# lich0031/AIDE

Hardware: AMD Instinct MI355X
Metric: training images/sec FuseUNet 256x256x2 bs=4/GPU (higher is better)
Workload: dtype f32; 1 GPU; c2 fuseunet fwd+loss+bwd+Adam(amsgrad), 256x256 2-modal, bs=4/GPU, fp32; global_batch=4, parallelism=dp1

## Files before the change

aide_amd/csrc/conv3x3_wino4.hip:

```cpp
#include "common.h"
#include <stdlib.h>
#include <type_traits>

namespace {

template <int V> using ic = std::integral_constant<int, V>;

__device__ __forceinline__ void buf_store_f32x4(f32x4 v, __amdgpu_buffer_rsrc_t r, unsigned voff, unsigned soff) {
    __builtin_amdgcn_raw_buffer_store_b128(__builtin_bit_cast(u32x4, v), r, voff, soff, 0);
}
__device__ __forceinline__ void buf_store_f32x2(f32x2 v, __amdgpu_buffer_rsrc_t r, unsigned voff, unsigned soff) {
    __builtin_amdgcn_raw_buffer_store_b64(__builtin_bit_cast(u32x2, v), r, voff, soff, 0);
}

struct W4Args {
    const float* x;
    const float* u;
    const float* bias;
    float* y;
    long x_bs, y_bs, split_stride;
    int N, Cin, H, W, Cout;
    int blocks_w, blocks_h, n_co_tiles, splitk, stages_total, accumulate;
    int gp, gc;
    int pair;
    float* stats;
    const float* scale;
    int relu;
    const float* in_tab;
    int in_ng;
};

constexpr int F4_BNIN_MAXC = 1024;
constexpr int F4_NAGPR = 16;
constexpr int F4_RRS = 41;
constexpr int F4_RCS = 775;
constexpr int F4_RAW = 4 * F4_RCS;
constexpr int F4_V = 36 * 32 * 4;
constexpr int F4_SET = F4_RAW + F4_V;
constexpr int F4_LDS = 2 * F4_SET > 4 * 128 * 64 ? 2 * F4_SET : 4 * 128 * 64;

__host__ __device__ constexpr int f4_pos(int q, int b) {
    return 6 * (q / 3) + ((q % 3) == 0 ? 1 + b : (q % 3) == 1 ? 3 + b : 5 * b);
}
__host__ __device__ constexpr int f4_slot(int c) { return c == 0 ? 4 : c == 5 ? 5 : c - 1; }

__device__ __forceinline__ void bt6(float d0, float d1, float d2, float d3, float d4, float d5, float* o, int st) {
    const float a = __builtin_fmaf(-4.f, d2, d4), b = __builtin_fmaf(4.f, d1, -d3);
    const float c = d4 - d2, e = d3 - d1;
    o[0] = __builtin_fmaf(-5.f, d2, __builtin_fmaf(4.f, d0, d4));
    o[st] = a - b;
    o[2 * st] = a + b;
    o[3 * st] = __builtin_fmaf(2.f, e, c);
    o[4 * st] = __builtin_fmaf(-2.f, e, c);
    o[5 * st] = __builtin_fmaf(-5.f, d3, __builtin_fmaf(4.f, d1, d5));
}

template <int CTRL, int ROW_MASK>
__device__ __forceinline__ float dpp_add(float v) {
    return v + __builtin_bit_cast(float, __builtin_amdgcn_update_dpp(0, __builtin_bit_cast(int, v), CTRL, ROW_MASK, 0xf, true));
}
__device__ __forceinline__ float half_total_dpp(float v) {
    v = dpp_add<0x111, 0xf>(v);
    v = dpp_add<0x112, 0xf>(v);
    v = dpp_add<0x114, 0xf>(v);
    v = dpp_add<0x118, 0xf>(v);
    v = dpp_add<0x142, 0xa>(v);
    return v;
}

template <int MODE, bool AFF = false, bool BNIN = false>
__global__ __launch_bounds__(256, 1) void conv3x3_wino4_kernel(const W4Args a) {
    extern __shared__ __attribute__((aligned(16))) float lds[];
    const int wid = __builtin_amdgcn_readfirstlane((int)threadIdx.x >> 6);
    const int ph = wid & 1, cb = wid >> 1;
    const int hs = wid >> 1;

    int b = xcd_remap(blockIdx.x, gridDim.x);
    const int p_in = b % a.gp;            b /= a.gp;
    const int co_in = b % a.gc;           b /= a.gc;
    const int ncg = a.n_co_tiles / a.gc;
    const int cog = b % ncg;              b /= ncg;
    const int split = b % a.splitk;       b /= a.splitk;
    const int co_tile = cog * a.gc + co_in;
    int pt = b * a.gp + p_in;
    const int tw = pt % a.blocks_w;       pt /= a.blocks_w;
    const int th = pt % a.blocks_h;
    const int n = pt / a.blocks_h;
    constexpr int PAIR = MODE == 1;
    constexpr bool canv = MODE == 2;
    constexpr int NR = canv ? 22 : 18, NI = canv ? 5 : 8, RRS = canv ? 29 : F4_RRS;
    constexpr int TPH = canv ? 20 : 16, TPW = canv ? 20 : 32;
    static_assert(NR * RRS <= F4_RCS, "raw channel plane");
    const int h0 = th * TPH, w0 = tw * TPW, co0 = co_tile * 64;
    const int HW = a.H * a.W;
    constexpr int pair = PAIR;

    const int sps = a.stages_total / a.splitk;
    const int s_begin = split * sps;
    const int s_end = min(s_begin + sps, a.stages_total);

    const __amdgpu_buffer_rsrc_t xrs =
        make_rsrc(a.x + (long)(pair ? 2 * n : n) * a.x_bs + (long)h0 * a.W + w0 - (a.W + 1));
    const long ubase = ((long)9 * ph * 2 * a.Cout + co0 + cb * 32) * 4;
    const __amdgpu_buffer_rsrc_t urs = __builtin_amdgcn_make_buffer_rsrc(
        const_cast<float*>(a.u + ubase), 0, (int)(((long)a.Cin * 36 * a.Cout - ubase) * 4), 0x00020000);
    const unsigned upos = (unsigned)a.Cout * 32u;
    const unsigned upos18 = 18u * upos;
    auto run = [&](auto HS) {
    int lane;
    asm volatile("; lane id, transform half %1\n\tv_mbcnt_lo_u32_b32 %0, -1, 0\n\tv_mbcnt_hi_u32_b32 %0, -1, %0"
                 : "=v"(lane) : "n"(decltype(HS)::value));
    const int tid = wid * 64 + lane;
    const int half = lane >> 5, j = lane & 31;
    constexpr int NUI = 4 * NR * NI, NUE = 4 * NR * 2;
    unsigned offB[3], ldsB[3], offC, ldsC;
    int tabB[3], tabC;
#pragma unroll
    for (int e = 0; e < 3; ++e) {
        int q = tid + e * 256;
        while (q >= NUI) q -= 256;
        const int c = q / (NR * NI), rem = q - c * (NR * NI), r = rem / NI, s4 = rem - r * NI;
        const int ih = h0 - 1 + r, iw = w0 + 4 * s4;
        const int imgB = pair && s4 >= 4;
        const bool ok = ih >= 0 && ih < a.H && (pair || iw < a.W);
        offB[e] = ok ? (unsigned)((long)imgB * a.x_bs + c * HW + r * a.W + 1 + 4 * (pair ? (s4 & 3) : s4)) * 4u : BUF_OOB;
        ldsB[e] = (unsigned)(c * F4_RCS + r * RRS + 4 + 4 * s4 + 2 * imgB);
        tabB[e] = F4_LDS + (ok ? 0 : 2 * a.Cin) + 2 * c;
    }
    {
        int q = tid;
        if (q >= NUE) q -= NUE;
        const int c = q / (NR * 2), rem = q - c * (NR * 2), r = rem >> 1, side = rem & 1;
        const int ih = h0 - 1 + r, iw = side ? w0 + TPW : w0 - 1;
        const bool ok = !pair && ih >= 0 && ih < a.H && iw >= 0 && iw < a.W;
        tabC = F4_LDS + (ok ? 0 : 2 * a.Cin) + 2 * c;
        offC = ok ? (unsigned)(c * HW + r * a.W + (side ? TPW + 1 : 0)) * 4u : BUF_OOB;
        ldsC = (unsigned)(c * F4_RCS + r * RRS + (pair ? (side ? 21 : 20) : (side ? 4 + TPW : 3)));
    }
#pragma unroll
    for (int e = 0; e < 3; ++e) asm volatile("" : "+v"(ldsB[e]), "+v"(offB[e]));
    asm volatile("" : "+v"(ldsC), "+v"(offC));
    const unsigned uoff = (unsigned)(half * a.Cout + j) * 16u;

    f32x4 rb[3];
    float rc;
    f32x4 ua[2][9];
    auto fetch_u = [&](int q, int stage, f32x4* dst) {
        const unsigned us = (unsigned)min(stage, s_end - 1) * upos18 + (unsigned)q * upos;
        dst[q] = buf_load_f32x4(urs, uoff, us);
    };
    auto fetch = [&](int l, int stage) {
        const unsigned xs = (unsigned)(min(stage, s_end - 1) * 4) * (unsigned)HW * 4u;
        if (l < 3) rb[l] = buf_load_f32x4(xrs, offB[l], xs);
        else rc = buf_load_f32(xrs, offC, xs);
    };
    auto put_raw = [&](int w, float* raw) {
        if (w < 12) raw[ldsB[w >> 2] + (w & 3)] = rb[w >> 2][w & 3];
        else raw[ldsC] = rc;
    };
    f32x2 tv[4];
    auto bn_tab = [&](int stage) {
        const int so = min(stage, s_end - 1) * 8;
#pragma unroll
        for (int e = 0; e < 3; ++e) tv[e] = *reinterpret_cast<const f32x2*>(lds + tabB[e] + so);
        tv[3] = *reinterpret_cast<const f32x2*>(lds + tabC + so);
    };
    auto bn_in = [&]() {
#pragma unroll
        for (int e = 0; e < 3; ++e) {
            const f32x2 sc = f32x2{tv[e].x, tv[e].x}, sh = f32x2{tv[e].y, tv[e].y};
            const f32x2 lo = f32x2{rb[e].x, rb[e].y} * sc + sh, hi = f32x2{rb[e].z, rb[e].w} * sc + sh;
            rb[e] = f32x4{fmaxf(lo.x, 0.f), fmaxf(lo.y, 0.f), fmaxf(hi.x, 0.f), fmaxf(hi.y, 0.f)};
        }
        rc = fmaxf(__builtin_fmaf(rc, tv[3].x, tv[3].y), 0.f);
    };
    if constexpr (BNIN) {
        float* tab = lds + F4_LDS;
        const float* src = a.in_tab + (long)(n / a.in_ng) * 2 * a.Cin;
        for (int i = tid; i < 2 * a.Cin; i += 256) { tab[i] = src[i]; tab[2 * a.Cin + i] = 0.f; }
        __syncthreads();
    }

    const int item = tid & 127;
    const int tslot = canv ? min(item >> 2, 24) : (item >> 2);
    const int trow = canv ? tslot / 5 : tslot >> 3, tcol = canv ? tslot - 5 * trow : tslot & 7;
    const int xr_off = (item & 3) * F4_RCS + trow * 4 * RRS + 3 + 4 * tcol + ((pair && tcol >= 4) ? 2 : 0);
    f32x2 tp[6][3];
    f32x2 tq[9];
    auto xf_read = [&](int i, int xo) {
        const float v = lds[xo + (i / 6) * RRS + (i % 6)];
        if ((i % 6) & 1) tp[i / 6][(i % 6) >> 1].y = v; else tp[i / 6][(i % 6) >> 1].x = v;
    };
    auto xf_half = [&](auto HS) {
        constexpr int khs = decltype(HS)::value;
        f32x2 T[3][3];
#pragma unroll
        for (int cp = 0; cp < 3; ++cp) {
            const f32x2 d0 = tp[0][cp], d1 = tp[1][cp], d2 = tp[2][cp], d3 = tp[3][cp], d4 = tp[4][cp], d5 = tp[5][cp];
            if (khs == 0) {
                const f32x2 aa = d4 - 4.f * d2, bb = 4.f * d1 - d3;
                T[0][cp] = (4.f * d0 + d4) - 5.f * d2;
                T[1][cp] = bb * f32x2{-1.f, -1.f} + aa;
                T[2][cp] = aa + bb;
            } else {
                const f32x2 cc = d2 * f32x2{-1.f, -1.f} + d4, ee = d1 * f32x2{-1.f, -1.f} + d3;
                T[0][cp] = cc + 2.f * ee;
                T[1][cp] = cc - 2.f * ee;
                T[2][cp] = (4.f * d1 + d5) - 5.f * d3;
            }
        }
#pragma unroll
        for (int i = 0; i < 3; ++i) {
            const f32x2 t01 = T[i][0], t23 = T[i][1], t45 = T[i][2];
            const f32x2 ac = f32x2{t23.x, t23.x} * f32x2{-4.f, -1.f} + f32x2{t45.x, t45.x};
            const f32x2 be = f32x2{t01.y, t01.y} * f32x2{-4.f, -1.f} + f32x2{t23.y, t23.y};
            const f32x2 o12 = f32x2{be.x, be.x} * f32x2{1.f, -1.f} + f32x2{ac.x, ac.x};
            const f32x2 o34 = f32x2{be.y, be.y} * f32x2{2.f, -2.f} + f32x2{ac.y, ac.y};
            const f32x2 o05 = t23 * f32x2{-5.f, -5.f} + (t01 * f32x2{4.f, 4.f} + t45);
            tq[3 * i] = o12; tq[3 * i + 1] = o34; tq[3 * i + 2] = o05;
        }
    };
    auto xf_math = [&]() { xf_half(HS); };
    const int vitem = ((item >> 1) & 1) * 128 + ((((item >> 2) * 4 + (item & 1) * 2)) ^ (((item >> 1) & 1) * 16));
    auto xf_store = [&](int m, float* vbuf) {
        *reinterpret_cast<f32x2*>(vbuf + (9 * hs + m) * 256 + vitem) = tq[m];
    };

    f32x16 acc[18];
    f32x4 fb[3];

    float* const set0 = lds;
    float* const set1 = lds + F4_SET;
    int xr0 = xr_off, xr1 = F4_SET + xr_off;
    asm volatile("" : "+v"(xr0), "+v"(xr1));
#pragma unroll
    for (int l = 0; l < 4; ++l) fetch(l, s_begin);
#pragma unroll
    for (int q = 0; q < 9; ++q) fetch_u(q, s_begin, ua[0]);
    __builtin_amdgcn_sched_barrier(0);
#pragma unroll
    for (int p = 0; p < 18; ++p) {
#pragma unroll
        for (int r = 0; r < 16; ++r) {
            float z;
            if (p < F4_NAGPR) asm volatile("v_accvgpr_write_b32 %0, 0" : "=a"(z));
            else asm volatile("v_mov_b32 %0, 0" : "=v"(z));
            acc[p][r] = z;
        }
    }
    __builtin_amdgcn_sched_barrier(0);
    if (pair) {
        for (int q = tid; q < 2 * 4 * 18 * 2; q += 256) {
            const int set = q / 144, rem = q - set * 144, c = rem / 36, rr = (rem % 36) >> 1, side = rem & 1;
            lds[set * F4_SET + c * F4_RCS + rr * F4_RRS + (side ? 38 : 3)] = 0.f;
        }
    }
    if constexpr (BNIN) { bn_tab(s_begin); bn_in(); }
#pragma unroll
    for (int w = 0; w < 13; ++w) put_raw(w, set0);
#pragma unroll
    for (int l = 0; l < 4; ++l) fetch(l, s_begin + 1);
    __syncthreads();
#pragma unroll
    for (int i = 0; i < 36; ++i) xf_read(i, xr0);
    xf_math();
#pragma unroll
    for (int m = 0; m < 9; ++m) xf_store(m, set0 + F4_RAW);
    if constexpr (BNIN) { bn_tab(s_begin + 1); bn_in(); }
#pragma unroll
    for (int w = 0; w < 13; ++w) put_raw(w, set1);
    __syncthreads();

    auto stage = [&](int s, float* sc, float* sn, auto CUR) {
        constexpr int kcur = decltype(CUR)::value;
        const float* lb = sc + F4_RAW + (9 * ph) * 256 + half * 128 + ((j * 4) ^ (half * 16));
        auto frag = [&](int q, int slot3) { fb[slot3] = *reinterpret_cast<const f32x4*>(lb + q * 256); };
        frag(0, 0); frag(1, 1);
#pragma unroll
        for (int st = 0; st < 36; ++st) {
            const int g = st >> 2, w = st & 3, pi = 2 * g + (w & 1), k = w >> 1;
            const int fs = g % 3;
            if (w == 0 && g + 2 < 9) frag(g + 2, (g + 2) % 3);
            if (pi < F4_NAGPR) asm volatile("v_mfma_f32_32x32x2_f32 %0, %1, %2, %0" : "+a"(acc[pi]) : "v"(ua[kcur][g][(w & 1) * 2 + k]), "v"(fb[fs][k * 2 + (w & 1)]));
            else asm volatile("v_mfma_f32_32x32x2_f32 %0, %1, %2, %0" : "+v"(acc[pi]) : "v"(ua[kcur][g][(w & 1) * 2 + k]), "v"(fb[fs][k * 2 + (w & 1)]));
            if (st < 4) fetch(st, s + 2);
            else if (st < 22 && ((st - 4) & 1) == 0) fetch_u((st - 4) >> 1, s + 1, ua[1 - kcur]);
            constexpr int XM = 20, XS = 21, PR = 31;
            if (st < 18) { xf_read(2 * st, kcur ? xr0 : xr1); xf_read(2 * st + 1, kcur ? xr0 : xr1); }
            if (st == XM) xf_math();
            if (st >= XS && st < XS + 9) xf_store(st - XS, sn + F4_RAW);
            if constexpr (BNIN) {
                if (st == 24) bn_tab(s + 2);
                if (st == 30) bn_in();
            }
            if (st >= PR && st < PR + 5) {
#pragma unroll
                for (int q = 0; q < 3; ++q)
                    if (3 * (st - PR) + q < 13) put_raw(3 * (st - PR) + q, sc);
            }
            __builtin_amdgcn_sched_barrier(0);
        }
        __syncthreads();
    };
    for (int s = s_begin; s < s_end; s += 2) {
        stage(s, set0, set1, ic<0>{});
        stage(s + 1, set1, set0, ic<1>{});
    }

    float* xbuf = lds;
    const int el = (int)__builtin_amdgcn_mbcnt_hi(~0u, __builtin_amdgcn_mbcnt_lo(~0u, 0u));
    const int eh = el >> 5, ej = el & 31;
    int ez;
    asm volatile("s_mov_b32 %0, 0" : "=s"(ez));
    const int cw = co0 + cb * 32 + ez;
    const bool wlive = cw < a.Cout;
    const bool add_bias = (a.bias != nullptr) && (split == 0);
    const __amdgpu_buffer_rsrc_t yrs = __builtin_amdgcn_make_buffer_rsrc(
        a.y + (long)split * a.split_stride + (long)(pair ? 2 * n : n) * a.y_bs + ez, 0, wlive ? (int)BUF_OOB : 0, 0x00020000);
    const __amdgpu_buffer_rsrc_t brs = __builtin_amdgcn_make_buffer_rsrc(
        const_cast<float*>(a.bias) + ez, 0, (add_bias && wlive) ? a.Cout * 4 : 0, 0x00020000);
    const int oh = h0 + 4 * (canv ? ej / 5 : ej >> 3), ow = pair ? 4 * (ej & 3) : w0 + 4 * (canv ? ej % 5 : ej & 7);
    const bool pok = (!canv || ej < 25) && oh < a.H && ow < a.W;
    const unsigned yoff = pok ? ((pair ? (unsigned)((ej & 7) >> 2) * (unsigned)a.y_bs : 0u) +
                                 (unsigned)(4 * eh * HW + oh * a.W + ow)) * 4u : BUF_OOB;
    const unsigned boff = (unsigned)eh * 16u;
    const int nparts = a.N * a.blocks_h * a.blocks_w;
    const __amdgpu_buffer_rsrc_t srs = __builtin_amdgcn_make_buffer_rsrc(
        a.stats + ez, 0, (a.stats != nullptr && wlive) ? a.Cout * nparts * 8 : 0, 0x00020000);
    const unsigned soff = ej == 31 ? (unsigned)(4 * eh * nparts + (n * a.blocks_h + th) * a.blocks_w + tw) * 8u : BUF_OOB;
    auto epilogue = [&](auto PH) {
        constexpr int kph = decltype(PH)::value;
        auto partial = [&](int r, f32x2* yp) {
            f32x2 T[3][4];
#pragma unroll
            for (int i = 0; i < 3; ++i) {
                auto m = [&](int c) { return f32x2{acc[6 * i + f4_slot(c)][r], acc[6 * i + f4_slot(c)][r + 1]}; };
                const f32x2 m0 = m(0), m1 = m(1), m2 = m(2), m3 = m(3), m4 = m(4), m5 = m(5);
                const f32x2 s12 = m1 + m2, d12 = m2 * f32x2{-1.f, -1.f} + m1, s34 = m3 + m4, d34 = m4 * f32x2{-1.f, -1.f} + m3;
                T[i][0] = m0 + s12 + s34;
                T[i][1] = d34 * f32x2{2.f, 2.f} + d12;
                T[i][2] = s34 * f32x2{4.f, 4.f} + s12;
                T[i][3] = d34 * f32x2{8.f, 8.f} + d12 + m5;
            }
#pragma unroll
            for (int bq = 0; bq < 4; ++bq) {
                if (kph == 0) {
                    const f32x2 sm = T[1][bq] + T[2][bq], df = T[2][bq] * f32x2{-1.f, -1.f} + T[1][bq];
                    yp[bq] = T[0][bq] + sm; yp[4 + bq] = df; yp[8 + bq] = sm; yp[12 + bq] = df;
                } else {
                    const f32x2 sm = T[0][bq] + T[1][bq], df = T[1][bq] * f32x2{-1.f, -1.f} + T[0][bq];
                    yp[bq] = sm; yp[4 + bq] = df * f32x2{2.f, 2.f}; yp[8 + bq] = sm * f32x2{4.f, 4.f};
                    yp[12 + bq] = df * f32x2{8.f, 8.f} + T[2][bq];
                }
            }
        };
        f32x2* const xbuf2 = reinterpret_cast<f32x2*>(xbuf);
#pragma unroll
        for (int rp = 0; rp < 4; ++rp) {
            f32x2 yp[16];
            partial(2 * rp + 8 * (1 - kph), yp);
#pragma unroll
            for (int o = 0; o < 16; ++o) xbuf2[((wid * 64) + rp * 16 + o) * 64 + el] = yp[o];
        }
        float bvs[8], svs[8];
#pragma unroll
        for (int q = 0; q < 8; ++q) {
            const int r = q + 8 * kph;
            bvs[q] = buf_load_f32(brs, boff, (unsigned)(cw + (r & 3) + 8 * (r >> 2)) * 4u);
        }
        if constexpr (AFF) {
            const __amdgpu_buffer_rsrc_t ars = __builtin_amdgcn_make_buffer_rsrc(const_cast<float*>(a.scale), 0, wlive ? a.Cout * 4 : 0, 0x00020000);
#pragma unroll
            for (int q = 0; q < 8; ++q) {
                const int r = q + 8 * kph;
                svs[q] = buf_load_f32(ars, boff, (unsigned)(cw + (r & 3) + 8 * (r >> 2)) * 4u);
            }
        }
        __syncthreads();
#pragma unroll
        for (int rp = 0; rp < 4; ++rp) {
            f32x2 yp[16];
            partial(2 * rp + 8 * kph, yp);
#pragma unroll
            for (int o = 0; o < 16; ++o) yp[o] += xbuf2[(((wid ^ 1) * 64) + rp * 16 + o) * 64 + el];
#pragma unroll
            for (int e = 0; e < 2; ++e) {
                const int r = 2 * rp + e + 8 * kph;
                const unsigned crow = (unsigned)(cw + (r & 3) + 8 * (r >> 2));
                if (a.stats) {
                    float s1 = 0.f, s2 = 0.f;
                    if (pok) {
#pragma unroll
                        for (int o = 0; o < 16; ++o) { s1 += yp[o][e]; s2 = __builtin_fmaf(yp[o][e], yp[o][e], s2); }
                    }
                    s1 = half_total_dpp(s1);
                    s2 = half_total_dpp(s2);
                    buf_store_f32x2(f32x2{s1, s2}, srs, soff, crow * (unsigned)nparts * 8u);
                }
                const float bv = bvs[2 * rp + e];
                const unsigned srow = crow * (unsigned)HW * 4u;
                f32x4 o[4];
#pragma unroll
                for (int i = 0; i < 4; ++i)
                    o[i] = f32x4{yp[4 * i][e] + bv, yp[4 * i + 1][e] + bv, yp[4 * i + 2][e] + bv, yp[4 * i + 3][e] + bv};
                if constexpr (AFF) {
                    const float sv = svs[2 * rp + e];
#pragma unroll
                    for (int i = 0; i < 4; ++i) {
#pragma unroll
                        for (int k = 0; k < 4; ++k) {
                            const float v = __builtin_fmaf(yp[4 * i + k][e], sv, bv);
                            o[i][k] = a.relu ? fmaxf(v, 0.f) : v;
                        }
                    }
                }
                if (a.accumulate) {
                    f32x4 old[4];
#pragma unroll
                    for (int i = 0; i < 4; ++i) old[i] = buf_load_f32x4(yrs, yoff, srow + (unsigned)(i * a.W) * 4u);
#pragma unroll
                    for (int i = 0; i < 4; ++i) o[i] += old[i];
                }
#pragma unroll
                for (int i = 0; i < 4; ++i) buf_store_f32x4(o[i], yrs, yoff, srow + (unsigned)(i * a.W) * 4u);
            }
        }
    };
    if (ph == 0) epilogue(ic<0>{}); else epilogue(ic<1>{});
    };
    if (hs == 0) run(ic<0>{}); else run(ic<1>{});
}

__global__ __launch_bounds__(256) void w4_splitk_reduce_kernel(const float* __restrict__ slabs, long split_stride,
                                                               int splitk, float* __restrict__ y, long y_bs, int C,
                                                               int HW, const float* __restrict__ bias, int accumulate,
                                                               long total4, const float* __restrict__ scale, int relu) {
    for (long i = (long)blockIdx.x * 256 + threadIdx.x; i < total4; i += (long)gridDim.x * 256) {
        const long e = i * 4, chw = (long)C * HW;
        const long n = e / chw, rem = e - n * chw;
        f32x4 v = *reinterpret_cast<const f32x4*>(slabs + e);
        for (int s = 1; s < splitk; ++s) v += *reinterpret_cast<const f32x4*>(slabs + (long)s * split_stride + e);
        if (scale) {
            const float sv = scale[rem / HW], bv = bias[rem / HW];
#pragma unroll
            for (int k = 0; k < 4; ++k) { const float t = __builtin_fmaf(v[k], sv, bv); v[k] = relu ? fmaxf(t, 0.f) : t; }
        } else if (bias) { const float bv = bias[rem / HW]; v += f32x4{bv, bv, bv, bv}; }
        f32x4* p = reinterpret_cast<f32x4*>(y + n * y_bs + rem);
        if (accumulate) v += *p;
        *p = v;
    }
}

__device__ __forceinline__ void wino4_g(const float g[9], float u[36]) {
    float t[18];
#pragma unroll
    for (int c = 0; c < 3; ++c) {
        const float g0 = g[c], g1 = g[3 + c], g2 = g[6 + c];
        const float s = g0 + g2;
        t[c] = 0.25f * g0;
        t[3 + c] = (-1.f / 6.f) * (s + g1);
        t[6 + c] = (-1.f / 6.f) * (s - g1);
        const float q = __builtin_fmaf(4.f, g2, g0);
        t[9 + c] = (1.f / 24.f) * (q + 2.f * g1);
        t[12 + c] = (1.f / 24.f) * (q - 2.f * g1);
        t[15 + c] = g2;
    }
#pragma unroll
    for (int r = 0; r < 6; ++r) {
        const float a0 = t[r * 3], a1 = t[r * 3 + 1], a2 = t[r * 3 + 2];
        const float s = a0 + a2, q = __builtin_fmaf(4.f, a2, a0);
        u[r * 6] = 0.25f * a0;
        u[r * 6 + 1] = (-1.f / 6.f) * (s + a1);
        u[r * 6 + 2] = (-1.f / 6.f) * (s - a1);
        u[r * 6 + 3] = (1.f / 24.f) * (q + 2.f * a1);
        u[r * 6 + 4] = (1.f / 24.f) * (q - 2.f * a1);
        u[r * 6 + 5] = a2;
    }
}

struct W4PackDesc {
    const float* w; float* uf; float* ud;
    int Co, Ci, pad0, pad1;
    long block_start;
};

constexpr int P4_T = 32;
__global__ __launch_bounds__(128) void wino4_pack_multi_kernel(const W4PackDesc* __restrict__ descs, int n, long total_blocks) {
    __shared__ __attribute__((aligned(16))) float ot[36 * 128];
    for (long blk = blockIdx.x; blk < total_blocks; blk += gridDim.x) {
    int lo = 0, hi = n - 1;
    while (lo < hi) {
        const int mid = (lo + hi + 1) >> 1;
        if (descs[mid].block_start <= blk) lo = mid; else hi = mid - 1;
    }
    const W4PackDesc d = descs[lo];
    const int tid = threadIdx.x;
    const int tiles_ci = (d.Ci + P4_T - 1) / P4_T;
    const int tb = (int)(blk - d.block_start);
    const int co0 = (tb / tiles_ci) * P4_T, ci0 = (tb % tiles_ci) * P4_T;
    const int nci = min(P4_T, d.Ci - ci0);
    float g[9], u[36];
    const int lo2 = tid & 3, hi5 = tid >> 2;
    for (int grp = 0; grp < 16; ++grp) {
        const bool fwd = grp < 8;
        const int q = grp & 7;
        float* dst = fwd ? d.uf : d.ud;
        if (dst == nullptr) continue;
        const int co = fwd ? hi5 : 4 * q + lo2, ci = fwd ? 4 * q + lo2 : hi5;
        const bool live = fwd ? (ci0 + 4 * q < d.Ci) : (co0 + 4 * q < d.Co);
        if (!live) continue;
        {
            const bool in = co0 + co < d.Co && ci < nci;
            const float* wp = d.w + ((long)(co0 + co) * d.Ci + ci0 + ci) * 9;
#pragma unroll
            for (int t = 0; t < 9; ++t) g[t] = in ? wp[fwd ? t : 8 - t] : 0.f;
        }
        wino4_g(g, u);
        const int otid = (lo2 >> 1) * 64 + hi5 * 2 + (lo2 & 1);
#pragma unroll
        for (int p = 0; p < 36; ++p) ot[p * 128 + otid] = u[p];
        __syncthreads();
        const int C = fwd ? d.Co : d.Ci, c0 = fwd ? co0 : ci0;
        const long gbase = (long)((fwd ? ci0 : co0) / 4 + q) * 18;
        const int nrow = min(P4_T, C - c0);
#pragma unroll
        for (int k = 0; k < 9; ++k) {
            const int f = tid + k * 128, pq = f >> 6, hh = (f >> 5) & 1, row = f & 31;
            if (row < nrow) {
                const float* o0 = ot + f4_pos(pq, 0) * 128 + hh * 64 + row * 2;
                const float* o1 = ot + f4_pos(pq, 1) * 128 + hh * 64 + row * 2;
                *reinterpret_cast<f32x4*>(dst + (((gbase + pq) * 2 + hh) * C + c0 + row) * 4) =
                    f32x4{o0[0], o0[1], o1[0], o1[1]};
            }
        }
        __syncthreads();
    }
    }
}

}

extern "C" {

int aide_conv3x3_wino4_supported(int Cin, int H, int W, int Cout) {
    return (H % 4 == 0 && W % 4 == 0 && H >= 16 && W >= 16 && Cout % 32 == 0 &&
            Cin % 8 == 0) ? 1 : 0;
}

static int f4_mode(int H, int W, int* bh, int* bw) {
    const int sh = (H + 15) / 16, sw = (W + 31) / 32, ch = (H + 19) / 20, cw = (W + 19) / 20;
    const int mode = W == 16 ? 1 : ((long)ch * cw < (long)sh * sw) ? 2 : 0;
    *bh = mode == 2 ? ch : sh;
    *bw = mode == 2 ? cw : sw;
    return mode;
}

int aide_conv3x3_wino4_splitk(int N, int Cin, int H, int W, int Cout) {
    int bh, bw;
    f4_mode(H, W, &bh, &bw);
    const long nb = (long)bh * bw * (W == 16 ? N / 2 : N) * ((Cout + 63) / 64);
    const int pairs = Cin / 8;
    const long target = 200;
    int s = 1;
    while (nb * s < target && pairs % (s * 2) == 0 && s * 2 <= pairs / 4) s *= 2;
    return s;
}

int aide_conv3x3_wino4_stats_parts(int N, int H, int W) {
    int bh, bw;
    f4_mode(H, W, &bh, &bw);
    return W < 32 ? 0 : N * bh * bw;
}

int aide_conv3x3_wino4_pack_blocks(int Co, int Ci) {
    return ((Co + P4_T - 1) / P4_T) * ((Ci + P4_T - 1) / P4_T);
}

int aide_conv3x3_wino4_pack_multi(const void* descs, int n, int64_t total_blocks, hipStream_t stream) {
    if (!descs || n <= 0 || total_blocks <= 0) return AIDE_ERR_ARG;
    static_assert(sizeof(W4PackDesc) == 48, "descriptor layout");
    const long grid = total_blocks;
    AIDE_LAUNCH_TIMED(AIDE_KT_OTHER, 0.0, wino4_pack_multi_kernel, dim3((unsigned)grid), dim3(128), 0, stream,
                       (const W4PackDesc*)descs, n, (long)total_blocks);
    return aide_launch_status();
}

int aide_conv3x3_wino4(const float* x, int64_t x_bs, const float* u, const float* bias, float* y,
                       int64_t y_bs, int N, int Cin, int H, int W, int Cout, int accumulate, int splitk,
                       float* ws, float* stats_parts, const float* epi_scale, int epi_relu, const float* in_bn_tab,
                       int in_bn_group_images, hipStream_t stream) {
    const float* aff = epi_scale;
    const int aff_relu = aff ? epi_relu : 0;
    if (!x || !u || !y || !aide_conv3x3_wino4_supported(Cin, H, W, Cout) || x_bs % 4 || y_bs % 4 || (W == 16 && N % 2))
        return AIDE_ERR_ARG;
    static AideLdsOptIn lds_opt;
    if (int rc = lds_opt.ensure([] {
            constexpr int plain = F4_LDS * (int)sizeof(float), bnin = (F4_LDS + 4 * F4_BNIN_MAXC) * (int)sizeof(float);
            const struct { const void* fn; int bytes; } ks[] = {
                {(const void*)conv3x3_wino4_kernel<0>, plain}, {(const void*)conv3x3_wino4_kernel<1>, plain},
                {(const void*)conv3x3_wino4_kernel<2>, plain}, {(const void*)conv3x3_wino4_kernel<0, true>, plain},
                {(const void*)conv3x3_wino4_kernel<2, true>, plain}, {(const void*)conv3x3_wino4_kernel<0, false, true>, bnin},
                {(const void*)conv3x3_wino4_kernel<2, false, true>, bnin}};
            for (const auto& k : ks) {
                const hipError_t e = hipFuncSetAttribute(k.fn, hipFuncAttributeMaxDynamicSharedMemorySize, k.bytes);
                if (e != hipSuccess) return e;
            }
            return hipSuccess;
        })) return rc;
    W4Args a;
    if (stats_parts && !(splitk <= 1 && accumulate == 0 && W >= 32)) return AIDE_ERR_ARG;
    a.stats = stats_parts;
    const int mode = f4_mode(H, W, &a.blocks_h, &a.blocks_w);
    if (aff && (accumulate != 0 || !bias || (mode == 1 && splitk <= 1))) return AIDE_ERR_ARG;
    a.scale = splitk > 1 ? nullptr : aff;
    a.relu = aff_relu;
    a.pair = mode == 1 ? 1 : 0;
    if (in_bn_tab && (mode == 1 || aff || Cin > F4_BNIN_MAXC || in_bn_group_images < 1 || N % in_bn_group_images)) return AIDE_ERR_ARG;
    a.in_tab = in_bn_tab; a.in_ng = in_bn_tab ? in_bn_group_images : 1;
    a.x = x; a.u = u; a.x_bs = x_bs; a.N = N; a.Cin = Cin; a.H = H; a.W = W; a.Cout = Cout;
    a.n_co_tiles = (Cout + 63) / 64;
    a.stages_total = Cin / 4;
    if (splitk < 1) splitk = 1;
    if ((Cin / 8) % splitk != 0) return AIDE_ERR_ARG;
    if (splitk > 1 && !ws) return AIDE_ERR_ARG;
    a.splitk = splitk;
    if (splitk > 1) {
        a.y = ws; a.y_bs = (long)Cout * H * W; a.split_stride = (long)N * Cout * H * W;
        a.bias = nullptr; a.accumulate = 0;
    } else {
        a.y = y; a.y_bs = y_bs; a.split_stride = 0; a.bias = bias; a.accumulate = (accumulate == 1);
    }
    if (((a.pair ? a.y_bs : 0) + (long)Cout * H * W) * 4 >= (1L << 31)) return AIDE_ERR_ARG;
    if (a.stats && (long)Cout * N * a.blocks_h * a.blocks_w * 8 >= (1L << 31)) return AIDE_ERR_ARG;
    const long nb = (long)a.blocks_w * a.blocks_h * (a.pair ? N / 2 : N) * a.n_co_tiles * splitk;
    {
        const long P = (long)a.blocks_w * a.blocks_h * (a.pair ? N / 2 : N);
        const int C = a.n_co_tiles;
        const long per_xcd = nb / 8 > 0 ? nb / 8 : 1;
        const double ub = 144.0 * (double)Cin * Cout, xb = 1.44 * 4.0 * (double)N * Cin * H * W;
        long bp = 1; int bc = C;
        double best = 1e300;
        const bool grouped = AIDE_CONV_FLOPS(N, H, W, Cout, Cin) >= 8e9;
        for (long gp = 1; gp <= P && gp <= per_xcd && grouped; gp *= 2) {
            if (P % gp) continue;
            for (int gc = 1; gc <= C; ++gc) {
                if (C % gc || gp * gc > per_xcd) continue;
                const double cost = ub * (double)P / (double)gp + xb * (double)C / (double)gc;
                if (cost < best) { best = cost; bp = gp; bc = gc; }
            }
        }
        a.gp = (int)bp; a.gc = bc;
    }
    if (a.in_tab) {
        const size_t lds_bytes = (F4_LDS + 4 * (size_t)Cin) * sizeof(float);
        if (mode == 2) {
            AIDE_LAUNCH_TIMED(AIDE_KT_WINO4, AIDE_CONV_FLOPS(N, H, W, Cout, Cin), (conv3x3_wino4_kernel<2, false, true>),
                              dim3((unsigned)nb), dim3(256), lds_bytes, stream, a);
        } else {
            AIDE_LAUNCH_TIMED(AIDE_KT_WINO4, AIDE_CONV_FLOPS(N, H, W, Cout, Cin), (conv3x3_wino4_kernel<0, false, true>),
                              dim3((unsigned)nb), dim3(256), lds_bytes, stream, a);
        }
    } else if (a.scale && mode == 2) {
        AIDE_LAUNCH_TIMED(AIDE_KT_WINO4, AIDE_CONV_FLOPS(N, H, W, Cout, Cin), (conv3x3_wino4_kernel<2, true>), dim3((unsigned)nb),
                          dim3(256), F4_LDS * sizeof(float), stream, a);
    } else if (a.scale) {
        AIDE_LAUNCH_TIMED(AIDE_KT_WINO4, AIDE_CONV_FLOPS(N, H, W, Cout, Cin), (conv3x3_wino4_kernel<0, true>), dim3((unsigned)nb),
                          dim3(256), F4_LDS * sizeof(float), stream, a);
    } else if (a.pair) {
        AIDE_LAUNCH_TIMED(AIDE_KT_WINO4, AIDE_CONV_FLOPS(N, H, W, Cout, Cin), conv3x3_wino4_kernel<1>, dim3((unsigned)nb), dim3(256),
                          F4_LDS * sizeof(float), stream, a);
    } else if (mode == 2) {
        AIDE_LAUNCH_TIMED(AIDE_KT_WINO4, AIDE_CONV_FLOPS(N, H, W, Cout, Cin), conv3x3_wino4_kernel<2>, dim3((unsigned)nb), dim3(256),
                          F4_LDS * sizeof(float), stream, a);
    } else {
        AIDE_LAUNCH_TIMED(AIDE_KT_WINO4, AIDE_CONV_FLOPS(N, H, W, Cout, Cin), conv3x3_wino4_kernel<0>, dim3((unsigned)nb), dim3(256),
                          F4_LDS * sizeof(float), stream, a);
    }
    int rc = aide_launch_status();
    if (rc != 0) return rc;
    if (splitk > 1 && accumulate != 2) {
        const long total4 = (long)N * Cout * H * W / 4;
        AIDE_LAUNCH_TIMED(AIDE_KT_REDUCE, 0.0, w4_splitk_reduce_kernel, dim3((unsigned)min((total4 + 255) / 256, 4096L)), dim3(256), 0,
                           stream, ws, (long)N * Cout * H * W, splitk, y, (long)y_bs, Cout, H * W, bias, accumulate,
                           total4, aff, aff_relu);
        rc = aide_launch_status();
    }
    return rc;
}

}
```

Baseline: 655.6 images/sec.

## Move stage barrier inside the Winograd MFMA loop and prefetch next-stage fragments

Restructures the software pipeline of the F(4,3) Winograd conv kernel. The per-stage __syncthreads now sits at slot 31 of the 36-slot MFMA schedule instead of at the end. The first two V fragments of the next stage are loaded after that barrier, so MFMAs can keep issuing across the stage boundary. Raw-input global fetches move later and run three stages ahead, and raw LDS stores and BN steps are rescheduled earlier, with static_asserts checking the slot ordering. This hides the barrier and fragment-load latency at the cost of more register pressure and a deeper global prefetch, whose out-of-range stage index must be handled safely.

```diff
diff --git a/aide_amd/csrc/conv3x3_wino4.hip b/aide_amd/csrc/conv3x3_wino4.hip
--- a/aide_amd/csrc/conv3x3_wino4.hip
+++ b/aide_amd/csrc/conv3x3_wino4.hip
@@ -38,6 +38,49 @@
 constexpr int F4_V = 36 * 32 * 4;
 constexpr int F4_SET = F4_RAW + F4_V;
 constexpr int F4_LDS = 2 * F4_SET > 4 * 128 * 64 ? 2 * F4_SET : 4 * 128 * 64;
+
+constexpr int W4_SLOTS = 36, W4_PAIRS = 9;
+constexpr int W4_FB = 3;
+constexpr int W4_AHEAD = 2;
+constexpr int W4_XR = 0, W4_XR_N = 18;
+constexpr int W4_UF = 4;
+constexpr int W4_XM = 20;
+constexpr int W4_XS = 21;
+constexpr int W4_BT = 19, W4_BI = 23;
+constexpr int W4_PR = 24, W4_PR_N = 5;
+constexpr int W4_RF = 29, W4_RF_N = 4;
+constexpr int W4_BAR = 31;
+constexpr int W4_PF0 = 31, W4_PF1 = 32;
+constexpr int w4_frag_slot(int q) { return 4 * (q - W4_AHEAD); }
+constexpr int w4_last_use(int g) { return 4 * g + 3; }
+constexpr int w4_last_pair_of(int f) {
+    int g = -1;
+    for (int q = 0; q < W4_PAIRS; ++q) if (q % W4_FB == f) g = q;
+    return g;
+}
+constexpr bool w4_fb_rotation_ok() {
+    for (int q = W4_AHEAD; q < W4_PAIRS; ++q) {
+        if (w4_frag_slot(q) < 0 || w4_frag_slot(q) >= 4 * q) return false;
+        if (q >= W4_FB && w4_frag_slot(q) <= w4_last_use(q - W4_FB)) return false;
+    }
+    return true;
+}
+static_assert(W4_BAR > 0 && W4_BAR < W4_SLOTS, "one barrier per stage, inside it");
+static_assert(w4_frag_slot(W4_PAIRS - 1) < W4_BAR, "sc.V is read in front of the barrier: the next interval overwrites it");
+static_assert(W4_PF0 >= W4_BAR && W4_PF1 >= W4_BAR && W4_PF0 < W4_SLOTS && W4_PF1 < W4_SLOTS,
+              "sn.V is read behind the barrier that follows its stores");
+static_assert(W4_XS >= W4_XM && W4_XS + W4_PAIRS - 1 < W4_BAR, "sn.V is written in front of the barrier");
+static_assert(W4_XR >= 0 && W4_XR + W4_XR_N - 1 < W4_BAR, "sn.raw is read in front of the barrier: the next interval overwrites it");
+static_assert(W4_PR >= 0 && W4_PR + W4_PR_N - 1 < W4_BAR, "sc.raw is written in front of the barrier, its readers follow behind it");
+static_assert(3 * W4_PR_N >= 13 && 2 * W4_XR_N == 36, "13 raw words, 36 patch words per thread");
+static_assert(W4_XM > W4_XR + W4_XR_N - 1, "the transform follows the last patch read");
+static_assert(W4_RF > W4_PR + W4_PR_N - 1 && W4_RF + W4_RF_N <= W4_SLOTS, "the raw registers are refilled behind their LDS stores");
+static_assert(W4_BT < W4_BI && W4_BI <= W4_PR && W4_BI != W4_XM, "BNIN: table, then the activation, then the raw stores");
+static_assert(W4_UF + 2 * (W4_PAIRS - 1) < W4_RF, "nine filter fetches per stage, in slots of their own");
+static_assert(W4_AHEAD == 2 && W4_FB == 3 && w4_fb_rotation_ok(), "fragment q: requested at slot 4 (q - 2) into fb[q % 3]");
+static_assert(W4_PF0 > w4_last_use(w4_last_pair_of(0)) && W4_PF1 > w4_last_use(w4_last_pair_of(1)),
+              "the next stage's fragments 0 / 1 go into fb[0] / fb[1] behind the last pair that used them");
+static_assert(W4_PF0 != W4_PF1, "one prefetch per slot");
 
 __host__ __device__ constexpr int f4_pos(int q, int b) {
     return 6 * (q / 3) + ((q % 3) == 0 ? 1 + b : (q % 3) == 1 ? 3 + b : 5 * b);
@@ -227,12 +270,14 @@
     };
 
     f32x16 acc[18];
-    f32x4 fb[3];
+    f32x4 fb[W4_FB];
 
     float* const set0 = lds;
     float* const set1 = lds + F4_SET;
     int xr0 = xr_off, xr1 = F4_SET + xr_off;
     asm volatile("" : "+v"(xr0), "+v"(xr1));
+    const int vfrag = (9 * ph) * 256 + half * 128 + ((j * 4) ^ (half * 16));
+    auto frag = [&](int q, const float* set) { fb[q % W4_FB] = *reinterpret_cast<const f32x4*>(set + F4_RAW + vfrag + q * 256); };
 #pragma unroll
     for (int l = 0; l < 4; ++l) fetch(l, s_begin);
 #pragma unroll
@@ -269,43 +314,48 @@
     if constexpr (BNIN) { bn_tab(s_begin + 1); bn_in(); }
 #pragma unroll
     for (int w = 0; w < 13; ++w) put_raw(w, set1);
+#pragma unroll
+    for (int l = 0; l < 4; ++l) fetch(l, s_begin + 2);
     __syncthreads();
+#pragma unroll
+    for (int q = 0; q < W4_AHEAD; ++q) frag(q, set0);
 
     auto stage = [&](int s, float* sc, float* sn, auto CUR) {
         constexpr int kcur = decltype(CUR)::value;
-        const float* lb = sc + F4_RAW + (9 * ph) * 256 + half * 128 + ((j * 4) ^ (half * 16));
-        auto frag = [&](int q, int slot3) { fb[slot3] = *reinterpret_cast<const f32x4*>(lb + q * 256); };
-        frag(0, 0); frag(1, 1);
-#pragma unroll
-        for (int st = 0; st < 36; ++st) {
+#pragma unroll
+        for (int st = 0; st < W4_SLOTS; ++st) {
             const int g = st >> 2, w = st & 3, pi = 2 * g + (w & 1), k = w >> 1;
-            const int fs = g % 3;
-            if (w == 0 && g + 2 < 9) frag(g + 2, (g + 2) % 3);
+            const int fs = g % W4_FB;
+            if (st == W4_BAR) __syncthreads();
+            if (w == 0 && g + W4_AHEAD < W4_PAIRS) frag(g + W4_AHEAD, sc);
+            if (st == W4_PF0) frag(0, sn);
+            if (st == W4_PF1) frag(1, sn);
             if (pi < F4_NAGPR) asm volatile("v_mfma_f32_32x32x2_f32 %0, %1, %2, %0" : "+a"(acc[pi]) : "v"(ua[kcur][g][(w & 1) * 2 + k]), "v"(fb[fs][k * 2 + (w & 1)]));
             else asm volatile("v_mfma_f32_32x32x2_f32 %0, %1, %2, %0" : "+v"(acc[pi]) : "v"(ua[kcur][g][(w & 1) * 2 + k]), "v"(fb[fs][k * 2 + (w & 1)]));
-            if (st < 4) fetch(st, s + 2);
-            else if (st < 22 && ((st - 4) & 1) == 0) fetch_u((st - 4) >> 1, s + 1, ua[1 - kcur]);
-            constexpr int XM = 20, XS = 21, PR = 31;
-            if (st < 18) { xf_read(2 * st, kcur ? xr0 : xr1); xf_read(2 * st + 1, kcur ? xr0 : xr1); }
-            if (st == XM) xf_math();
-            if (st >= XS && st < XS + 9) xf_store(st - XS, sn + F4_RAW);
+            if (st >= W4_RF && st < W4_RF + W4_RF_N) fetch(st - W4_RF, s + 3);
+            else if (st >= W4_UF && st < W4_UF + 2 * W4_PAIRS && ((st - W4_UF) & 1) == 0) fetch_u((st - W4_UF) >> 1, s + 1, ua[1 - kcur]);
+            if (st >= W4_XR && st < W4_XR + W4_XR_N) {
+                xf_read(2 * (st - W4_XR), kcur ? xr0 : xr1); xf_read(2 * (st - W4_XR) + 1, kcur ? xr0 : xr1);
+            }
+            if (st == W4_XM) xf_math();
+            if (st >= W4_XS && st < W4_XS + W4_PAIRS) xf_store(st - W4_XS, sn + F4_RAW);
             if constexpr (BNIN) {
-                if (st == 24) bn_tab(s + 2);
-                if (st == 30) bn_in();
-            }
-            if (st >= PR && st < PR + 5) {
+                if (st == W4_BT) bn_tab(s + 2);
+                if (st == W4_BI) bn_in();
+            }
+            if (st >= W4_PR && st < W4_PR + W4_PR_N) {
 #pragma unroll
                 for (int q = 0; q < 3; ++q)
-                    if (3 * (st - PR) + q < 13) put_raw(3 * (st - PR) + q, sc);
+                    if (3 * (st - W4_PR) + q < 13) put_raw(3 * (st - W4_PR) + q, sc);
             }
             __builtin_amdgcn_sched_barrier(0);
         }
-        __syncthreads();
     };
     for (int s = s_begin; s < s_end; s += 2) {
         stage(s, set0, set1, ic<0>{});
         stage(s + 1, set1, set0, ic<1>{});
     }
+    __syncthreads();
 
     float* xbuf = lds;
     const int el = (int)__builtin_amdgcn_mbcnt_hi(~0u, __builtin_amdgcn_mbcnt_lo(~0u, 0u));
```

After: 659.7 images/sec, median of 6. No clear change (+0.6%).
